# silverlight6/Ultrasound_Modeling

Hardware: AMD Instinct MI355X
Metric: segmentation training images/sec at 256x256 (higher is better)
Workload: dtype bf16

## Files before the change

ultrasound_modeling_amd/csrc/conv_big.hip:

```cpp
#include "common.h"

struct BigJob {
  const bf16_t* x;
  const bf16_t* w;
  void* y;
  const float* bias;
  const float* scale;
  const bf16_t* res;
  int32_t H, W, d, Hl, Wl, PH, PW, NV;
  int32_t tiles_x, tiles_per_v, npatches;
  int32_t ldx, ldy, ldr, Cin, nchunks, Nw, Kw, Nout, act;
  float alpha;
  int32_t out_f32, accumulate, flip;
  int32_t gx, gy, npa, nstages;
  uint32_t x_bytes, w_bytes;
  int32_t mask_ch;
  int32_t one_tap;
  uint16_t tapmask[4];
};
struct BigParams {
  BigJob job[4];
};

typedef __attribute__((address_space(3))) void* lds_ptr_t;
#define OOB_OFF 0x80000000u

template <int NT, int NS, int NW = 4>
__global__ __launch_bounds__(64 * NW) void conv_big_kernel(const BigParams P) {
#if defined(__HIP_DEVICE_COMPILE__)
  constexpr int BN = 16 * NT;
  constexpr int W_BYTES = 9 * BN * 64;
  constexpr int NPW = 9 * BN / 16;
  constexpr int W_IT = (NPW + NW - 1) / NW;
  constexpr int A_IT = ((NS * NW == 16 ? 36 : 18) + NW - 1) / NW;
  extern __shared__ __attribute__((aligned(1024))) char lds[];
  const BigJob& p = P.job[blockIdx.z];
  if ((int)blockIdx.x >= p.gx || (int)blockIdx.y >= p.gy) return;

  const int tid = threadIdx.x, lane = tid & 63, wv = __builtin_amdgcn_readfirstlane(tid >> 6);
  const int n0 = blockIdx.y * BN;
  const int HW2 = p.PW + 2, HPP = (p.PH + 2) * HW2, NHP = p.NV * HPP;
  const int a_bytes = p.npa * 1024, stage_bytes = a_bytes + W_BYTES;
  const int dd = p.d * p.d;
  const float r_hpp = fdiv_rcp(HPP), r_hw2 = fdiv_rcp(HW2), r_tpv = fdiv_rcp(p.tiles_per_v), r_tx = fdiv_rcp(p.tiles_x), r_dd = fdiv_rcp(dd),
              r_d = fdiv_rcp(p.d);

  const __amdgpu_buffer_rsrc_t rx = __builtin_amdgcn_make_buffer_rsrc((void*)p.x, 0, p.x_bytes, 0x00020000);
  const __amdgpu_buffer_rsrc_t rw = __builtin_amdgcn_make_buffer_rsrc((void*)p.w, 0, p.w_bytes, 0x00020000);
  const int slot_q = (lane & 3) ^ (((lane >> 4) & 1) << 1);
  uint32_t a_off[A_IT], w_off[W_IT];
#pragma unroll
  for (int it = 0; it < A_IT; ++it) {
    const int hp = 16 * (wv + NW * it) + (lane >> 2);
    uint32_t off = OOB_OFF;
    if (hp < NHP) {
      int pi, rem, hy, hx;
      fdivmod(hp, HPP, r_hpp, pi, rem);
      fdivmod(rem, HW2, r_hw2, hy, hx);
      int gp = blockIdx.x * p.NV + pi;
      if (gp < p.npatches) {
        int v, tt, ty, tx, b, ab, la, lb;
        fdivmod(gp, p.tiles_per_v, r_tpv, v, tt);
        fdivmod(tt, p.tiles_x, r_tx, ty, tx);
        fdivmod(v, dd, r_dd, b, ab);
        fdivmod(ab, p.d, r_d, la, lb);
        int ly = __mul24(ty, p.PH) + hy - 1, lx = __mul24(tx, p.PW) + hx - 1;
        if ((unsigned)ly < (unsigned)p.Hl && (unsigned)lx < (unsigned)p.Wl)
          off = (uint32_t)(__mul24(__mul24(__mul24(b, p.H) + la + __mul24(p.d, ly), p.W) + lb + __mul24(p.d, lx), p.ldx) + slot_q * 8) * 2u;
      }
    }
    a_off[it] = off;
  }
#pragma unroll
  for (int it = 0; it < W_IT; ++it) {
    const int row = 16 * (wv + NW * it) + (lane >> 2);
    uint32_t off = OOB_OFF;
    if (row < 9 * BN) {
      int t = row / BN, n = row - t * BN;
      int tw = p.flip ? 8 - t : t;
      if (p.one_tap) tw = t == 4 ? 0 : -1;
      if (tw >= 0 && n0 + n < p.Nw) off = (uint32_t)((n0 + n) * p.Kw + tw * p.Cin + slot_q * 8) * 2u;
    }
    w_off[it] = off;
  }
  const int cq = slot_q * 8;

  auto issue = [&](int ck, int stage) {
    char* abuf = lds + stage * stage_bytes;
    char* wbuf = abuf + a_bytes;
    const uint32_t cb = ck * 64;
    const bool cok = ck * 32 + cq < p.Cin;
#pragma unroll
    for (int it = 0; it < A_IT; ++it) {
      const int j = wv + NW * it;
      if (j < p.npa) {
        __builtin_amdgcn_raw_ptr_buffer_load_lds(rx, (lds_ptr_t)(abuf + j * 1024), 16, cok ? a_off[it] + cb : OOB_OFF, 0, 0, 0);
      }
    }
#pragma unroll
    for (int it = 0; it < W_IT; ++it) {
      const int j = wv + NW * it;
      if (j < NPW) {
        __builtin_amdgcn_raw_ptr_buffer_load_lds(rw, (lds_ptr_t)(wbuf + j * 1024), 16, cok ? w_off[it] + cb : OOB_OFF, 0, 0, 0);
      }
    }
  };

  issue(0, 0);
  const int pl = lane & 15, qk = lane >> 4;
  const int rows_per_strip = 16 / p.PW, spp = (p.PH * p.PW) >> 4;
  int hb[NS];
  int64_t opix[NS];
  bool ovalid[NS];
#pragma unroll
  for (int a = 0; a < NS; ++a) {
    int s = wv * NS + a;
    int pi, sl, r, c;
    fdivmod(s, spp, fdiv_rcp(spp), pi, sl);
    fdivmod(pl, p.PW, fdiv_rcp(p.PW), r, c);
    int row = sl * rows_per_strip + r;
    hb[a] = pi * HPP + row * HW2 + c;
    int gp = blockIdx.x * p.NV + pi;
    ovalid[a] = gp < p.npatches;
    int gpc = ovalid[a] ? gp : 0;
    int v, tt, ty, tx, b, ab, la, lb;
    fdivmod(gpc, p.tiles_per_v, r_tpv, v, tt);
    fdivmod(tt, p.tiles_x, r_tx, ty, tx);
    fdivmod(v, dd, r_dd, b, ab);
    fdivmod(ab, p.d, r_d, la, lb);
    int iy = la + __mul24(p.d, __mul24(ty, p.PH) + row), ix = lb + __mul24(p.d, __mul24(tx, p.PW) + c);
    opix[a] = (int64_t)(__mul24(__mul24(b, p.H) + iy, p.W) + ix);
  }
  const int w_lane = pl * 64 + ((qk ^ (((pl >> 2) & 1) << 1)) << 4);

  f32x4_t acc[NS][NT];
#pragma unroll
  for (int a = 0; a < NS; ++a)
#pragma unroll
    for (int b = 0; b < NT; ++b) acc[a][b] = (f32x4_t){0.f, 0.f, 0.f, 0.f};

  const bool dbuf = p.nstages == 2;
  for (int ck = 0; ck < p.nchunks; ++ck) {
    asm volatile("s_waitcnt vmcnt(0)" ::: "memory");
    __syncthreads();
    if (dbuf && ck + 1 < p.nchunks) issue(ck + 1, (ck + 1) & 1);
    const char* abuf = lds + (dbuf ? (ck & 1) * stage_bytes : 0);
    const char* wbuf = abuf + a_bytes + w_lane;
    const uint32_t tmask = p.one_tap ? 0x010u : (p.mask_ch ? p.tapmask[(p.flip ? ck * 32 : n0) / p.mask_ch] : 0x1ffu);
#pragma unroll
    for (int t = 0; t < 9; ++t) {
      if (!((tmask >> t) & 1u)) continue;
      const int toff = (t / 3) * HW2 + (t % 3);
      bf16x8_t xf[NS], wf[NT];
#pragma unroll
      for (int a = 0; a < NS; ++a) {
        const int hp = hb[a] + toff;
        xf[a] = *reinterpret_cast<const bf16x8_t*>(abuf + (hp << 6) + ((qk << 4) ^ ((hp & 4) << 3)));
      }
#pragma unroll
      for (int b = 0; b < NT; ++b) wf[b] = *reinterpret_cast<const bf16x8_t*>(wbuf + (t * BN + b * 16) * 64);
#pragma unroll
      for (int a = 0; a < NS; ++a)
#pragma unroll
        for (int b = 0; b < NT; ++b) acc[a][b] = __builtin_amdgcn_mfma_f32_16x16x32_bf16(wf[b], xf[a], acc[a][b], 0, 0, 0);
    }
    if (!dbuf && ck + 1 < p.nchunks) {
      __syncthreads();
      issue(ck + 1, 0);
    }
  }

  const EpiArgs e = {p.scale, p.bias, p.res, p.y, p.ldy, p.ldr, p.Nout, p.act, p.alpha, p.out_f32, p.accumulate};
  const int nbase = n0 + qk * 4;
  EpiConst<NT> ec;
  epi_const_load<NT>(ec, p.bias, nbase, p.Nout);
  conv_epilogue<NS, NT>(e, ec, acc, opix, ovalid, nbase);
#endif
}

template <int NT, int NS, bool RES = false>
__global__ __launch_bounds__(256, 2) void conv_stream_kernel(const BigParams P, const int fast_wait) {
#if defined(__HIP_DEVICE_COMPILE__)
  const BigJob& p = P.job[blockIdx.z];
  constexpr int BN = 16 * NT;
  constexpr int W_BYTES = 9 * BN * 64;
  constexpr int NPW = 9 * BN / 16;
  constexpr int A_IT = NS == 4 ? 6 : 3;
  constexpr int MAXG = 64;
  extern __shared__ __attribute__((aligned(1024))) char lds[];
  __shared__ int s_grp[MAXG][4];

  const int tid = threadIdx.x, lane = tid & 63, wv = __builtin_amdgcn_readfirstlane(tid >> 6);
  const int n0 = blockIdx.y * BN;
  const int HW2 = p.PW + 2, NHP = (p.PH + 2) * HW2;
  const int a_bytes = p.npa * 1024;
  char* const wlds = lds;
  char* const alds = lds + p.nchunks * W_BYTES;
  const int dd = p.d * p.d;
  const float r_nch = fdiv_rcp(p.nchunks);
  const float r_hw2 = fdiv_rcp(HW2), r_tpv = fdiv_rcp(p.tiles_per_v), r_tx = fdiv_rcp(p.tiles_x), r_dd = fdiv_rcp(dd), r_d = fdiv_rcp(p.d);

  const int ngroups = p.npatches;
  const int xcd = blockIdx.x & 7, wj = blockIdx.x >> 3, nj = gridDim.x >> 3;
  const int gpx = (ngroups + 7) >> 3;
  const int g_lo = xcd * gpx + wj;
  int g_hi = (xcd + 1) * gpx;
  if (g_hi > ngroups) g_hi = ngroups;
  int ng = g_lo < g_hi ? (g_hi - g_lo + nj - 1) / nj : 0;
  if (ng > MAXG) ng = MAXG;
  if (ng == 0) return;

  const __amdgpu_buffer_rsrc_t rx = __builtin_amdgcn_make_buffer_rsrc((void*)p.x, 0, p.x_bytes, 0x00020000);
  const __amdgpu_buffer_rsrc_t rw = __builtin_amdgcn_make_buffer_rsrc((void*)p.w, 0, p.w_bytes, 0x00020000);
  const int slot_q = (lane & 3) ^ (((lane >> 4) & 1) << 1);
  const int cq = slot_q * 8;

  for (int j = wv; j < p.nchunks * NPW; j += 4) {
    const int ck = j / NPW, r = j - ck * NPW;
    const int row = 16 * r + (lane >> 2);
    const int t = row / BN, n = row - t * BN;
    int tw = p.flip ? 8 - t : t;
    if (p.one_tap) tw = t == 4 ? 0 : -1;
    const bool ok = tw >= 0 && (n0 + n) < p.Nw && (ck * 32 + cq) < p.Cin;
    __builtin_amdgcn_raw_ptr_buffer_load_lds(rw, (lds_ptr_t)(wlds + j * 1024), 16,
                                             ok ? (uint32_t)((n0 + n) * p.Kw + tw * p.Cin + ck * 32 + cq) * 2u : OOB_OFF, 0, 0, 0);
  }
  for (int i = tid; i < ng; i += 256) {
    const int g = g_lo + i * nj;
    int v, tt, ty, tx, b, ab, la, lb;
    fdivmod(g, p.tiles_per_v, r_tpv, v, tt);
    fdivmod(tt, p.tiles_x, r_tx, ty, tx);
    fdivmod(v, dd, r_dd, b, ab);
    fdivmod(ab, p.d, r_d, la, lb);
    const int64_t org = (((int64_t)(b * p.H + la + p.d * (ty * p.PH - 1))) * p.W + lb + p.d * (tx * p.PW - 1)) * p.ldx * 2;
    s_grp[i][0] = (int)(uint32_t)org;
    s_grp[i][1] = (b * p.H + la + p.d * ty * p.PH) * p.W + lb + p.d * tx * p.PW;
    s_grp[i][2] = ty * p.PH - 1;
    s_grp[i][3] = tx * p.PW - 1;
  }
  uint32_t a_rel[A_IT];
  int a_hy[A_IT], a_hx[A_IT];
#pragma unroll
  for (int it = 0; it < A_IT; ++it) {
    const int hp = 16 * (wv + 4 * it) + (lane >> 2);
    int hy, hx;
    fdivmod(hp, HW2, r_hw2, hy, hx);
    a_hy[it] = hp < NHP ? hy : -(1 << 20);
    a_hx[it] = hx;
    a_rel[it] = (uint32_t)(((p.d * hy) * p.W + p.d * hx) * p.ldx + cq) * 2u;
  }
  const int pl = lane & 15, qk = lane >> 4;
  const int rows_per_strip = 16 / p.PW;
  int hb[NS], orel[NS];
#pragma unroll
  for (int a = 0; a < NS; ++a) {
    const int sl = wv * NS + a;
    int r, c;
    fdivmod(pl, p.PW, fdiv_rcp(p.PW), r, c);
    const int row = sl * rows_per_strip + r;
    hb[a] = row * HW2 + c;
    orel[a] = p.d * row * p.W + p.d * c;
  }
  const int w_lane = pl * 64 + ((qk ^ (((pl >> 2) & 1) << 1)) << 4);
  const EpiArgs e = {p.scale, p.bias, p.res, p.y, p.ldy, p.ldr, p.Nout, p.act, p.alpha, p.out_f32, p.accumulate};
  const int nbase = n0 + qk * 4;
  EpiConst<NT> ec;
  epi_const_load<NT>(ec, p.bias, nbase, p.Nout);
  __syncthreads();

  auto issue_a = [&](int s) {
    const int gl = __builtin_amdgcn_readfirstlane(fdiv(s, r_nch)), ck = s - gl * p.nchunks;
    char* abuf = alds + (s & 1) * a_bytes;
    const uint32_t org = (uint32_t)s_grp[gl][0] + ck * 64;
    const int lym1 = s_grp[gl][2], lxm1 = s_grp[gl][3];
    const bool cok = ck * 32 + cq < p.Cin;
#pragma unroll
    for (int it = 0; it < A_IT; ++it) {
      const int j = wv + 4 * it;
      if (j < p.npa) {
        const bool ok = cok && (unsigned)(lym1 + a_hy[it]) < (unsigned)p.Hl && (unsigned)(lxm1 + a_hx[it]) < (unsigned)p.Wl;
        __builtin_amdgcn_raw_ptr_buffer_load_lds(rx, (lds_ptr_t)(abuf + j * 1024), 16, ok ? org + a_rel[it] : OOB_OFF, 0, 0, 0);
      }
    }
  };

  f32x4_t acc[NS][NT];
  const int total = ng * p.nchunks;
  issue_a(0);
  for (int s = 0; s < total; ++s) {
    const int gl = __builtin_amdgcn_readfirstlane(fdiv(s, r_nch)), ck = s - gl * p.nchunks;
    if (fast_wait && s > 0 && ck == 0) asm volatile("s_waitcnt vmcnt(%0) lgkmcnt(0)\n\ts_barrier" ::"n"(NS * NT) : "memory");
    else asm volatile("s_waitcnt vmcnt(0) lgkmcnt(0)\n\ts_barrier" ::: "memory");
    uint2 rr[RES ? NS : 1][RES ? NT : 1];
    if constexpr (RES) {
      if (ck == p.nchunks - 1) {
        const int ob = s_grp[gl][1];
#pragma unroll
        for (int a = 0; a < NS; ++a)
#pragma unroll
          for (int b = 0; b < NT; ++b) {
            const int n = nbase + b * 16;
            rr[a][b] = *reinterpret_cast<const uint2*>(p.res + (int64_t)(ob + orel[a]) * p.ldr + (n < p.Nout ? n : 0));
          }
      }
    }
    if (s + 1 < total) issue_a(s + 1);
    if (ck == 0) {
#pragma unroll
      for (int a = 0; a < NS; ++a)
#pragma unroll
        for (int b = 0; b < NT; ++b) acc[a][b] = (f32x4_t){0.f, 0.f, 0.f, 0.f};
    }
    const char* abuf = alds + (s & 1) * a_bytes;
    const char* wbuf = wlds + ck * W_BYTES + w_lane;
    auto do_tap = [&](int t) {
      const int toff = (t / 3) * HW2 + (t % 3);
      bf16x8_t xf[NS], wf[NT];
#pragma unroll
      for (int a = 0; a < NS; ++a) {
        const int hp = hb[a] + toff;
        xf[a] = *reinterpret_cast<const bf16x8_t*>(abuf + (hp << 6) + ((qk << 4) ^ ((hp & 4) << 3)));
      }
#pragma unroll
      for (int b = 0; b < NT; ++b) wf[b] = *reinterpret_cast<const bf16x8_t*>(wbuf + (t * BN + b * 16) * 64);
#pragma unroll
      for (int a = 0; a < NS; ++a)
#pragma unroll
        for (int b = 0; b < NT; ++b) acc[a][b] = __builtin_amdgcn_mfma_f32_16x16x32_bf16(wf[b], xf[a], acc[a][b], 0, 0, 0);
    };
    if constexpr (RES || NT == 4) {
#pragma unroll
      for (int t = 0; t < 9; ++t) do_tap(t);
    } else if (p.one_tap) do_tap(4);
    else {
#pragma unroll
      for (int t = 0; t < 9; ++t) do_tap(t);
    }
    if (ck != p.nchunks - 1) continue;
    int64_t opix[NS];
    bool ovalid[NS];
    const int obase = s_grp[gl][1];
#pragma unroll
    for (int a = 0; a < NS; ++a) { opix[a] = obase + orel[a]; ovalid[a] = true; }
    if constexpr (RES) {
      const float alpha = p.alpha;
      const int act = p.act;
#pragma unroll
      for (int a = 0; a < NS; ++a) {
        bf16_t* const yrow = reinterpret_cast<bf16_t*>(p.y) + opix[a] * p.ldy;
#pragma unroll
        for (int b = 0; b < NT; ++b) {
          const int n = nbase + b * 16;
          if (n >= p.Nout) continue;
          const float v0 = apply_act(acc[a][b][0] + ec.bb[b].x, act, alpha) + __uint_as_float(rr[a][b].x << 16);
          const float v1 = apply_act(acc[a][b][1] + ec.bb[b].y, act, alpha) + __uint_as_float(rr[a][b].x & 0xffff0000u);
          const float v2 = apply_act(acc[a][b][2] + ec.bb[b].z, act, alpha) + __uint_as_float(rr[a][b].y << 16);
          const float v3 = apply_act(acc[a][b][3] + ec.bb[b].w, act, alpha) + __uint_as_float(rr[a][b].y & 0xffff0000u);
          uint2 o;
          o.x = pack2bf(v0, v1);
          o.y = pack2bf(v2, v3);
          *reinterpret_cast<uint2*>(yrow + n) = o;
        }
      }
    } else {
      conv_epilogue<NS, NT, true>(e, ec, acc, opix, ovalid, nbase);
    }
  }
#endif
}

static int big_fill_job(BigJob& p, const ConvPass& g, int PX, int any_cin = 0) {
  const int min_cin = knob<K_BIG_MIN_CIN>();
  const int B = g.B, H = g.H, W = g.W, d = g.d, ldx = g.ldx;
  if (d < 1 || H % d || W % d || (g.Cin < min_cin && !any_cin)) return 0;
  const int Hl = H / d, Wl = W / d;
  int PW;
  if (Wl % 16 == 0) PW = 16;
  else if (Wl == 8 || Wl == 4) PW = Wl;
  else return 0;
  int PH = PX / PW;
  if (PH > Hl) PH = Hl;
  if (Hl % PH || (PH * PW) % 16 || PX % (PH * PW)) return 0;
  const int NV = PX / (PH * PW);
  const int NHP = NV * (PH + 2) * (PW + 2);
  if (NHP > (PX == 256 ? 576 : 288)) return 0;
  if ((int64_t)B * H * W * ldx >= (1ll << 30) || (int64_t)g.Nw * g.Kw >= (1ll << 30)) return 0;
  if ((int64_t)B * H * W >= (1ll << 23) || (int64_t)B * d * d * (Hl / PH) * (Wl / PW) >= (1ll << 20)) return 0;
  p = {};
  p.x = g.x; p.w = g.w; p.y = g.y; p.bias = g.bias; p.scale = g.scale; p.res = g.res;
  p.H = H; p.W = W; p.d = d; p.Hl = Hl; p.Wl = Wl; p.PH = PH; p.PW = PW; p.NV = NV;
  p.tiles_x = Wl / PW;
  p.tiles_per_v = (Hl / PH) * p.tiles_x;
  p.npatches = B * d * d * p.tiles_per_v;
  p.ldx = ldx; p.ldy = g.ldy; p.ldr = g.ldr; p.Cin = g.Cin; p.nchunks = (g.Cin + 31) / 32;
  p.Nw = g.Nw; p.Kw = g.Kw; p.Nout = g.Nout; p.act = g.act; p.alpha = g.alpha; p.out_f32 = g.out_f32; p.accumulate = g.accumulate; p.flip = g.flip;
  p.gx = (p.npatches + NV - 1) / NV;
  p.x_bytes = (uint32_t)((int64_t)B * H * W * ldx * 2);
  p.w_bytes = (uint32_t)((int64_t)g.Nw * g.Kw * 2);
  p.npa = (NHP + 15) / 16;
  p.mask_ch = g.mask.group_ch;
  for (int c = 0; c < 4; ++c) p.tapmask[c] = g.mask.mask[c];
  p.one_tap = g.one_tap;
  return 1;
}

static int nt_for(int nout) { return nout <= 16 ? 1 : (nout <= 32 ? 2 : 4); }

template <int NT, int NS, int NW = 4>
static void big_launch_t(const BigParams& P, dim3 grid, size_t dyn, hipStream_t s) {
  if (usseg_lds_opt_in((const void*)conv_big_kernel<NT, NS, NW>, 160 * 1024)) return;
  hipLaunchKernelGGL((conv_big_kernel<NT, NS, NW>), grid, dim3(64 * NW), dyn, s, P);
}

static void big_launch(BigParams& P, int njobs, int nt, int PX, hipStream_t s, int w8 = 0) {
  int gx = 0, gy = 0, npa = 0;
  for (int j = 0; j < njobs; ++j) {
    BigJob& p = P.job[j];
    p.gy = (p.Nout + 16 * nt - 1) / (16 * nt);
    if (p.gx > gx) gx = p.gx;
    if (p.gy > gy) gy = p.gy;
    if (p.npa > npa) npa = p.npa;
  }
  const int stages_env = knob<K_BIG_STAGES>();
  int64_t total_wg = 0;
  for (int j = 0; j < njobs; ++j) total_wg += (int64_t)P.job[j].gx * P.job[j].gy;
  const int nstages = stages_env == 2 ? 2 : (stages_env == 1 ? 1 : (total_wg <= 512 ? 2 : 1));
  for (int j = 0; j < njobs; ++j) { P.job[j].npa = npa; P.job[j].nstages = nstages; }
  const size_t dyn = nstages * ((size_t)npa * 1024 + (size_t)9 * 16 * nt * 64);
  const dim3 grid(gx, gy, njobs);
  const int slot = usseg_prof_start(1, s);
  if (PX == 256 && w8) {
    if (nt == 1) big_launch_t<1, 2, 8>(P, grid, dyn, s);
    else if (nt == 2) big_launch_t<2, 2, 8>(P, grid, dyn, s);
    else big_launch_t<4, 2, 8>(P, grid, dyn, s);
  } else if (PX == 256) {
    if (nt == 1) big_launch_t<1, 4>(P, grid, dyn, s);
    else if (nt == 2) big_launch_t<2, 4>(P, grid, dyn, s);
    else big_launch_t<4, 4>(P, grid, dyn, s);
  } else {
    if (nt == 1) big_launch_t<1, 2>(P, grid, dyn, s);
    else if (nt == 2) big_launch_t<2, 2>(P, grid, dyn, s);
    else big_launch_t<4, 2>(P, grid, dyn, s);
  }
  usseg_prof_stop(1, slot, s);
}

template <int NT, int NS, bool RES = false>
static void stream_launch_t(const BigParams& P, dim3 grid, size_t dyn, int fast_wait, hipStream_t s) {
  if (usseg_lds_opt_in((const void*)conv_stream_kernel<NT, NS, RES>, 158 * 1024)) return;
  hipLaunchKernelGGL((conv_stream_kernel<NT, NS, RES>), grid, dim3(256), dyn, s, P, fast_wait);
}

struct StreamPlan {
  BigJob job;
  int nt, PX, res, fast_wait;
  size_t dyn;
  unsigned wgx, gy;
};
static int stream_plan(const ConvPass& g, StreamPlan& sp) {
  const int mode = knob<K_STREAM>();
  const int px_env = knob<K_STREAM_PX>();
  const int min_steps = knob<K_STREAM_MIN_STEPS>();
  const int wgx_env = knob<K_STREAM_WGX>();
  const int occ_env = knob<K_STREAM_OCC>();
  if (!mode || g.mask.group_ch) return 0;
  const int res_env = knob<K_STREAM_RES>();
  if (g.out_f32 || g.accumulate || g.scale) return 0;
  if (g.res && (!res_env || (g.ldr & 3))) return 0;
  const int nt = nt_for(g.Nout);
  const int nchunks = (g.Cin + 31) / 32;
  const size_t wbytes = (size_t)nchunks * 9 * 16 * nt * 64;
  if (wbytes > 40960) return 0;
  const int gy = (g.Nout + 16 * nt - 1) / (16 * nt);
  BigJob& p = sp.job;
  for (int PX = 256; PX >= 128; PX >>= 1) {
    if (px_env && PX != px_env) continue;
    if (!big_fill_job(p, g, PX, 1)) continue;
    if (p.NV != 1 || p.PW != 16) continue;
    if (g.one_tap && (nt == 4 || g.res)) return 0;
    const size_t dyn = wbytes + 2 * (size_t)p.npa * 1024;
    int occ = (int)((160 * 1024 - 2048) / (dyn + 1024));
    if (occ > 4) occ = 4;
    if (occ_env > 0 && occ_env < occ) occ = occ_env;
    if (occ < 1) continue;
    int wgx = (256 * occ / gy) & ~7;
    if (wgx < 8) wgx = 8;
    if (wgx_env >= 8) wgx = wgx_env & ~7;
    const int gpx = (p.npatches + 7) / 8;
    int per_wg = (gpx + wgx / 8 - 1) / (wgx / 8);
    if (per_wg * nchunks < min_steps && !px_env) continue;
    if (per_wg > 64) { wgx = ((gpx + 63) / 64) * 8; per_wg = 64; }
    sp.fast_wait = g.Nout % (16 * nt) == 0 && !g.res;
    sp.nt = nt; sp.PX = PX; sp.res = g.res != nullptr; sp.dyn = dyn; sp.wgx = (unsigned)wgx; sp.gy = (unsigned)gy;
    return 1;
  }
  return 0;
}
static void stream_launch(const StreamPlan* sp, int n, hipStream_t s) {
  BigParams P;
  for (int j = 0; j < n; ++j) P.job[j] = sp[j].job;
  for (int j = n; j < 4; ++j) P.job[j] = sp[0].job;
  const dim3 grid(sp[0].wgx, sp[0].gy, (unsigned)n);
  const int nt = sp[0].nt, PX = sp[0].PX, fast_wait = sp[0].fast_wait;
  const size_t dyn = sp[0].dyn;
  const int slot = usseg_prof_start(1, s);
  if (sp[0].res) {
    if (PX == 256) {
      if (nt == 1) stream_launch_t<1, 4, true>(P, grid, dyn, fast_wait, s);
      else if (nt == 2) stream_launch_t<2, 4, true>(P, grid, dyn, fast_wait, s);
      else stream_launch_t<4, 4, true>(P, grid, dyn, fast_wait, s);
    } else {
      if (nt == 1) stream_launch_t<1, 2, true>(P, grid, dyn, fast_wait, s);
      else if (nt == 2) stream_launch_t<2, 2, true>(P, grid, dyn, fast_wait, s);
      else stream_launch_t<4, 2, true>(P, grid, dyn, fast_wait, s);
    }
  } else if (PX == 256) {
    if (nt == 1) stream_launch_t<1, 4>(P, grid, dyn, fast_wait, s);
    else if (nt == 2) stream_launch_t<2, 4>(P, grid, dyn, fast_wait, s);
    else stream_launch_t<4, 4>(P, grid, dyn, fast_wait, s);
  } else {
    if (nt == 1) stream_launch_t<1, 2>(P, grid, dyn, fast_wait, s);
    else if (nt == 2) stream_launch_t<2, 2>(P, grid, dyn, fast_wait, s);
    else stream_launch_t<4, 2>(P, grid, dyn, fast_wait, s);
  }
  usseg_prof_stop(1, slot, s);
}
static bool stream_same_plan(const StreamPlan& a, const StreamPlan& b) {
  return a.nt == b.nt && a.PX == b.PX && a.res == b.res && a.fast_wait == b.fast_wait && a.dyn == b.dyn && a.wgx == b.wgx && a.gy == b.gy;
}

int usseg_try_launch_conv_big(const ConvPass* g, int njobs, hipStream_t s) {
  const int mode = knob<K_BIG>();
  const int px_env = knob<K_BIG_PX>();
  const int nt_env = knob<K_BIG_NT>();
  const int min_wg = knob<K_BIG_MIN_WG>();
  const int wg_min = knob<K_BIG_WG_TILE>();
  if (!mode || njobs < 1 || njobs > 4) return 0;
  {
    const int multi = knob<K_STREAM_MULTI>();
    const int merge = knob<K_STREAM_MERGE>();
    bool all = (njobs == 1 || multi) && njobs <= 4;
    StreamPlan sp[4];
    for (int j = 0; j < njobs && all; ++j) all = stream_plan(g[j], sp[j]) != 0;
    if (all) {
      for (int j = 0; j < njobs;) {
        int n = 1;
        while (merge && j + n < njobs && stream_same_plan(sp[j], sp[j + n])) ++n;
        stream_launch(sp + j, n, s);
        j += n;
      }
      return 1;
    }
  }
  int nt_max = 1;
  for (int j = 0; j < njobs; ++j) nt_max = nt_for(g[j].Nout) > nt_max ? nt_for(g[j].Nout) : nt_max;
  BigParams P;
  int best_px = 0, best_nt = 0;
  int64_t best_wg = 0;
  for (int PX = 256; PX >= 128 && !best_px; PX >>= 1) {
    if (px_env && PX != px_env) continue;
    bool ok = true;
    for (int j = 0; j < njobs && ok; ++j) ok = big_fill_job(P.job[j], g[j], PX);
    if (!ok) continue;
    for (int nt = nt_max; nt >= 1; nt >>= 1) {
      if (nt_env && nt != nt_env) continue;
      int64_t wg = 0;
      for (int j = 0; j < njobs; ++j) wg += (int64_t)P.job[j].gx * ((P.job[j].Nout + 16 * nt - 1) / (16 * nt));
      if (PX == 256 && !px_env) {
        if (nt == nt_max && wg >= 2048) { best_px = PX; best_nt = nt; best_wg = wg; }
        break;
      }
      best_px = PX; best_nt = nt; best_wg = wg;
      if (wg >= wg_min || nt_env) break;
    }
  }
  if (!best_px || (best_wg < min_wg && !(px_env || nt_env))) return 0;
  int w8 = 0;
  {
    const int w8_mode = knob<K_BIG_W8>();
    const int w8_min = knob<K_BIG_W8_MIN>();
    if (w8_mode && best_px == 128) {
      bool ok = true;
      int64_t wg = 0;
      for (int j = 0; j < njobs && ok; ++j) {
        ok = big_fill_job(P.job[j], g[j], 256);
        if (ok) wg += (int64_t)P.job[j].gx * ((P.job[j].Nout + 16 * best_nt - 1) / (16 * best_nt));
      }
      if (ok && ((wg >= w8_min && best_nt == 4) || w8_mode == 2)) { w8 = 1; best_px = 256; }
    }
  }
  for (int j = 0; j < njobs; ++j)
    if (!big_fill_job(P.job[j], g[j], best_px)) return 0;
  if (g[0].mask.group_ch && (njobs != 1 || g[0].mask.group_ch % (g[0].flip ? 32 : 16 * best_nt))) return 0;
  big_launch(P, njobs, best_nt, best_px, s, w8);
  return 1;
}
```

ultrasound_modeling_amd/csrc/knobs.h:

```cpp
#pragma once
#include <stdint.h>
#include <stdlib.h>

#define USSEG_KNOBS(X)                                                                                                                  \
                                                                                                                      \
  X(K_BIG,                "USSEG_BIG",                INT,     1,     ONCE,     "0: conv_big and the streaming conv take no launch")        \
  X(K_BIG_PX,             "USSEG_BIG_PX",             INT,     0,     ONCE,     "conv_big: force the pixel tile (128 / 256; 0: planner)")   \
  X(K_BIG_NT,             "USSEG_BIG_NT",             INT,     0,     ONCE,     "conv_big: force the channel tile (1 / 2 / 4 x 16; 0: planner)") \
  X(K_BIG_MIN_WG,         "USSEG_BIG_MIN_WG",         INT,     128,   ONCE,     "conv_big: smallest launch it takes, in workgroups")        \
  X(K_BIG_WG_TILE,        "USSEG_BIG_WG_TILE",        INT,     512,   ONCE,     "conv_big: narrow the channel tile below this many workgroups") \
  X(K_BIG_MIN_CIN,        "USSEG_BIG_MIN_CIN",        INT,     33,    ONCE,     "conv_big: fewest input channels of a pass it takes")       \
  X(K_BIG_STAGES,         "USSEG_BIG_STAGES",         INT,     0,     ONCE,     "conv_big LDS stages: 0 by launch size, 1 / 2 forced")      \
  X(K_BIG_W8,             "USSEG_BIG_W8",             INT,     1,     PER_CALL, "256-pixel tile on eight waves: 0 never, 1 planner, 2 forced") \
  X(K_BIG_W8_MIN,         "USSEG_BIG_W8_MIN",         INT,     128,   ONCE,     "fewest workgroups left for the eight-wave tile")           \
  X(K_STREAM,             "USSEG_STREAM",             INT,     1,     ONCE,     "0: the streaming conv takes no launch")                    \
  X(K_STREAM_PX,          "USSEG_STREAM_PX",          INT,     0,     ONCE,     "streaming conv: force the pixel tile (128 / 256; 0: planner)") \
  X(K_STREAM_MIN_STEPS,   "USSEG_STREAM_MIN_STEPS",   INT,     1,     PER_CALL, "streaming conv: fewest K steps per workgroup it takes")    \
  X(K_STREAM_WGX,         "USSEG_STREAM_WGX",         INT,     0,     PER_CALL, "streaming conv: force grid.x (>= 8, rounded down to a multiple of 8)") \
  X(K_STREAM_OCC,         "USSEG_STREAM_OCC",         INT,     0,     ONCE,     "streaming conv: cap on workgroups per CU (0: by LDS)")     \
  X(K_STREAM_RES,         "USSEG_STREAM_RES",         INT,     1,     ONCE,     "0: passes with a residual do not stream")                  \
  X(K_STREAM_MULTI,       "USSEG_STREAM_MULTI",       INT,     1,     ONCE,     "0: multi-job launches do not stream")                      \
  X(K_STREAM_MERGE,       "USSEG_STREAM_MERGE",       INT,     1,     PER_CALL, "streaming jobs of one plan in one launch (0: a launch per job)") \
                                                                                                     \
  X(K_NO_HALO,            "USSEG_NO_HALO",            PRESENT, 0,     ONCE,     "the halo-tile conv and weight-gradient kernels take no launch") \
  X(K_NO_PERSIST,         "USSEG_NO_PERSIST",         PRESENT, 0,     ONCE,     "conv_halo: never the persistent variant")                  \
  X(K_PERSIST_OCC,        "USSEG_PERSIST_OCC",        INT,     0,     ONCE,     "persistent conv_halo: workgroups per CU (0: by LDS)")      \
                                                                                                                    \
  X(K_IGEMM_WG_MIN,       "USSEG_IGEMM_WG_MIN",       INT,     256,   ONCE,     "igemm: narrow the channel tile below this many workgroups") \
  X(K_IGEMM_KC,           "USSEG_IGEMM_KC",           INT,     0,     ONCE,     "register-staged igemm: force the K step (4 / 8 chunks; 0: by K length)") \
  X(K_IGEMM_DMA,          "USSEG_IGEMM_DMA",          INT,     1,     ONCE,     "0: never the LDS-DMA igemm")                               \
  X(K_IGEMM_DMA_MIN,      "USSEG_IGEMM_DMA_MIN",      INT,     4,     ONCE,     "LDS-DMA igemm: fewest K chunks it takes")                  \
  X(K_IGEMM_DMA_BATCHED,  "USSEG_IGEMM_DMA_BATCHED",  INT,     1,     ONCE,     "0: batched GEMMs stay on the register-staged igemm")       \
  X(K_IGEMM_XCD,          "USSEG_IGEMM_XCD",          INT,     1,     ONCE,     "XCD-aware item order: 0 off, 1 activation-heavy launches, 2 all") \
  X(K_IGEMM_PERSIST,      "USSEG_IGEMM_PERSIST",      INT,     1,     ONCE,     "0: never the persistent LDS-DMA igemm")                    \
  X(K_IGEMM_STAGES8,      "USSEG_IGEMM_STAGES8",      INT,     4,     ONCE,     "ring depth of sparse long-K 128-channel launches (2: off, 3, 4)") \
  X(K_IGEMM_STAGES8_WG,   "USSEG_IGEMM_STAGES8_WG",   INT,     256,   ONCE,     "largest launch, in workgroups, that gets the deeper ring") \
                                                                                                         \
  X(K_WGRAD_DMA,          "USSEG_WGRAD_DMA",          INT,     1,     ONCE,     "0: never the LDS-DMA per-tap weight gradient / batched TN GEMM") \
  X(K_WGRAD_TM,           "USSEG_WGRAD_TM",           INT,     0,     ONCE,     "per-tap wgrad: force the tile (1: 64x64, 2: 128x128; 0: planner)") \
  X(K_WGD_TARGET,         "USSEG_WGD_TARGET",         INT,     512,   ONCE,     "per-tap wgrad: workgroups the split-K aims for")           \
  X(K_WGD_CAP,            "USSEG_WGD_CAP",            INT,     4,     ONCE,     "per-tap wgrad: slab traffic cap, in multiples of the operand bytes") \
  X(K_WG_QUANT,           "USSEG_WG_QUANT",           INT,     1,     ONCE,     "0: no wave-quantisation search of the split count (both wgrad kernels)") \
  X(K_WGRAD_DEBUG,        "USSEG_WGRAD_DEBUG",        PRESENT, 0,     ONCE,     "print every weight-gradient plan to stderr")               \
  X(K_WGRAD_POW2,         "USSEG_WGRAD_POW2",         INT,     1,     ONCE,     "0: no shift decode of power-of-two grids")                 \
  X(K_WGRAD_XCD,          "USSEG_WGRAD_XCD",          INT,     1,     ONCE,     "0: no XCD-aware item order in the per-tap wgrad")          \
  X(K_WG_TARGET,          "USSEG_WG_TARGET",          INT,     256,   ONCE,     "halo wgrad: workgroups the split-K aims for")              \
  X(K_SLAB_CAP,           "USSEG_SLAB_CAP",           INT,     2,     ONCE,     "halo wgrad: slab traffic cap, in multiples of the operand bytes") \
  X(K_WGHALO_XCD,         "USSEG_WGHALO_XCD",         INT,     1,     ONCE,     "0: no XCD-aware item order in the halo wgrad")             \
  X(K_WGRAD_PF,           "USSEG_WGRAD_PF",           INT,     1,     ONCE,     "0: halo wgrad without the register prefetch")              \
  X(K_WGRAD_8W,           "USSEG_WGRAD_8W",           INT,     1,     ONCE,     "0: the 64x64 halo wgrad tile on four waves, not eight")    \
  X(K_TCONV_HALO,         "USSEG_TCONV_HALO",         INT,     0,     PER_CALL, "1: transposed-conv wgrad as four parity-class halo jobs")  \
                                                                                                                      \
  X(K_CARD_BWD_G,         "USSEG_CARD_BWD_G",         INT,     0,     ONCE,     "fused cardinal backward: force the workgroup pairs (0: one resident wave)") \
  X(K_LN_TILE,            "USSEG_LN_TILE",            INT,     1,     ONCE,     "0: never the tile LayerNorm backward")                     \
  X(K_LN_PAIR,            "USSEG_LN_PAIR",            INT,     1,     ONCE,     "0: never the paired LayerNorm backward launch")            \
  X(K_LN_TILE_MIN,        "USSEG_LN_TILE_MIN",        INT,     32768, ONCE,     "fewest pixels for the tile / paired LayerNorm backward")   \
                                                                                     \
  X(K_FLASH_TILE,         "USSEG_FLASH_TILE",         INT,     -1,    ONCE,     "fused attention tiling 0 / 1 / 2 (-1: by problem size)")   \
  X(K_WINATTN_MFMA,       "USSEG_WINATTN_MFMA",       INT,     1,     ONCE,     "0: window attention without the MFMA kernels")             \
  X(K_LOSS_PPT,           "USSEG_LOSS_PPT",           INT,     4,     ONCE,     "softmax + loss kernel: pixels per thread")

enum Knob {
#define X(id, name, kind, def, life, doc) id,
  USSEG_KNOBS(X)
#undef X
};
enum { KNOB_INT, KNOB_PRESENT, KNOB_ONCE, KNOB_PER_CALL };
struct KnobDef { const char* name; int kind; int64_t def; int life; };
constexpr KnobDef kKnobs[] = {
#define X(id, name, kind, def, life, doc) {name, KNOB_##kind, def, KNOB_##life},
  USSEG_KNOBS(X)
#undef X
};

template <Knob K>
__attribute__((visibility("hidden"))) inline int64_t knob() {
  auto read = [] {
    const char* v = getenv(kKnobs[K].name);
    return kKnobs[K].kind == KNOB_PRESENT ? (int64_t)(v != nullptr) : (v ? (int64_t)atoll(v) : kKnobs[K].def);
  };
  if constexpr (kKnobs[K].life == KNOB_PER_CALL) return read();
  else {
    static const int64_t v = read();
    return v;
  }
}
```

Baseline: 5527.

## Prefetch LDS fragments ahead of MFMAs in narrow streaming conv tiles

Adds a software-pipelined path for the streaming conv kernel (non-residual, NT<=2). It preloads all nine tap weight fragments and a sliding window of input fragments, reusing input rows across kernel rows, and interleaves the LDS reads with MFMAs using sched_barriers. The aim is to hide LDS latency and cut redundant fragment reads. It uses more registers and could hurt occupancy. A default-on knob selects it.

```diff
diff --git a/ultrasound_modeling_amd/csrc/conv_big.hip b/ultrasound_modeling_amd/csrc/conv_big.hip
--- a/ultrasound_modeling_amd/csrc/conv_big.hip
+++ b/ultrasound_modeling_amd/csrc/conv_big.hip
@@ -1,3 +1,5 @@
+#include <type_traits>
+
 #include "common.h"
 
 struct BigJob {
@@ -179,7 +181,7 @@
 }
 
 template <int NT, int NS, bool RES = false>
-__global__ __launch_bounds__(256, 2) void conv_stream_kernel(const BigParams P, const int fast_wait) {
+__global__ __launch_bounds__(256, 2) void conv_stream_kernel(const BigParams P, const int fast_wait, const int frag_ahead) {
 #if defined(__HIP_DEVICE_COMPILE__)
   const BigJob& p = P.job[blockIdx.z];
   constexpr int BN = 16 * NT;
@@ -284,88 +286,143 @@
     }
   };
 
-  f32x4_t acc[NS][NT];
-  const int total = ng * p.nchunks;
-  issue_a(0);
-  for (int s = 0; s < total; ++s) {
-    const int gl = __builtin_amdgcn_readfirstlane(fdiv(s, r_nch)), ck = s - gl * p.nchunks;
-    if (fast_wait && s > 0 && ck == 0) asm volatile("s_waitcnt vmcnt(%0) lgkmcnt(0)\n\ts_barrier" ::"n"(NS * NT) : "memory");
-    else asm volatile("s_waitcnt vmcnt(0) lgkmcnt(0)\n\ts_barrier" ::: "memory");
-    uint2 rr[RES ? NS : 1][RES ? NT : 1];
-    if constexpr (RES) {
-      if (ck == p.nchunks - 1) {
-        const int ob = s_grp[gl][1];
+  constexpr bool AHEAD_OK = !RES && NT <= 2;
+  auto run = [&](auto ahead_c) {
+    constexpr bool AH = decltype(ahead_c)::value;
+    int xa[AH ? 4 : 1];
+    if constexpr (AH) {
+#pragma unroll
+      for (int m = 0; m < 4; ++m) {
+        const int hp = hb[0] + m;
+        xa[m] = (hp << 6) + ((qk << 4) ^ ((hp & 4) << 3));
+      }
+    }
+    f32x4_t acc[NS][NT];
+    const int total = ng * p.nchunks;
+    issue_a(0);
+    for (int s = 0; s < total; ++s) {
+      const int gl = __builtin_amdgcn_readfirstlane(fdiv(s, r_nch)), ck = s - gl * p.nchunks;
+      if (fast_wait && s > 0 && ck == 0) asm volatile("s_waitcnt vmcnt(%0) lgkmcnt(0)\n\ts_barrier" ::"n"(NS * NT) : "memory");
+      else asm volatile("s_waitcnt vmcnt(0) lgkmcnt(0)\n\ts_barrier" ::: "memory");
+      uint2 rr[RES ? NS : 1][RES ? NT : 1];
+      if constexpr (RES) {
+        if (ck == p.nchunks - 1) {
+          const int ob = s_grp[gl][1];
+#pragma unroll
+          for (int a = 0; a < NS; ++a)
+#pragma unroll
+            for (int b = 0; b < NT; ++b) {
+              const int n = nbase + b * 16;
+              rr[a][b] = *reinterpret_cast<const uint2*>(p.res + (int64_t)(ob + orel[a]) * p.ldr + (n < p.Nout ? n : 0));
+            }
+        }
+      }
+      if (s + 1 < total) issue_a(s + 1);
+      if (ck == 0) {
 #pragma unroll
         for (int a = 0; a < NS; ++a)
+#pragma unroll
+          for (int b = 0; b < NT; ++b) acc[a][b] = (f32x4_t){0.f, 0.f, 0.f, 0.f};
+      }
+      const int a_off = (s & 1) * a_bytes;
+      const char* abuf = alds + a_off;
+      const char* wbuf = wlds + ck * W_BYTES + w_lane;
+      auto do_tap = [&](int t) {
+        const int toff = (t / 3) * HW2 + (t % 3);
+        bf16x8_t xf[NS], wf[NT];
+#pragma unroll
+        for (int a = 0; a < NS; ++a) {
+          const int hp = hb[a] + toff;
+          xf[a] = *reinterpret_cast<const bf16x8_t*>(abuf + (hp << 6) + ((qk << 4) ^ ((hp & 4) << 3)));
+        }
+#pragma unroll
+        for (int b = 0; b < NT; ++b) wf[b] = *reinterpret_cast<const bf16x8_t*>(wbuf + (t * BN + b * 16) * 64);
+#pragma unroll
+        for (int a = 0; a < NS; ++a)
+#pragma unroll
+          for (int b = 0; b < NT; ++b) acc[a][b] = __builtin_amdgcn_mfma_f32_16x16x32_bf16(wf[b], xf[a], acc[a][b], 0, 0, 0);
+      };
+      if constexpr (RES || NT == 4) {
+#pragma unroll
+        for (int t = 0; t < 9; ++t) do_tap(t);
+      } else if (p.one_tap) do_tap(4);
+      else if constexpr (AH) {
+        bf16x8_t xf[NS + 2][3], wf[9][NT];
+        auto load_x = [&](int j, int kc) {
+          const int m = (2 * j + kc) & 7, off = a_off + xa[m & 3];
+          xf[j][kc] = *reinterpret_cast<const bf16x8_t*>(alds + (m < 4 ? off : off ^ 32) + 64 * (18 * j + kc - (m & 3)));
+        };
+        auto load_w = [&](int t) {
+#pragma unroll
+          for (int b = 0; b < NT; ++b) wf[t][b] = *reinterpret_cast<const bf16x8_t*>(wbuf + (t * BN + b * 16) * 64);
+        };
+#pragma unroll
+        for (int kc = 0; kc < 3; ++kc) {
+          load_w(kc);
+#pragma unroll
+          for (int j = 0; j < NS; ++j) load_x(j, kc);
+          __builtin_amdgcn_sched_barrier(0);
+        }
+#pragma unroll
+        for (int kr = 0; kr < 3; ++kr)
+#pragma unroll
+          for (int kc = 0; kc < 3; ++kc) {
+#pragma unroll
+            for (int a = 0; a < NS; ++a) {
+#pragma unroll
+              for (int b = 0; b < NT; ++b)
+                acc[a][b] = __builtin_amdgcn_mfma_f32_16x16x32_bf16(wf[kr * 3 + kc][b], xf[a + kr][kc], acc[a][b], 0, 0, 0);
+              if (a == 0 && kr < 2) {
+                __builtin_amdgcn_sched_barrier(0);
+                load_x(NS + kr, kc);
+                __builtin_amdgcn_sched_barrier(0);
+              }
+            }
+            if (kr < 2) {
+              __builtin_amdgcn_sched_barrier(0);
+              load_w(kr * 3 + kc + 3);
+              __builtin_amdgcn_sched_barrier(0);
+            }
+          }
+      } else {
+#pragma unroll
+        for (int t = 0; t < 9; ++t) do_tap(t);
+      }
+      if (ck != p.nchunks - 1) continue;
+      int64_t opix[NS];
+      bool ovalid[NS];
+      const int obase = s_grp[gl][1];
+#pragma unroll
+      for (int a = 0; a < NS; ++a) { opix[a] = obase + orel[a]; ovalid[a] = true; }
+      if constexpr (RES) {
+        const float alpha = p.alpha;
+        const int act = p.act;
+#pragma unroll
+        for (int a = 0; a < NS; ++a) {
+          bf16_t* const yrow = reinterpret_cast<bf16_t*>(p.y) + opix[a] * p.ldy;
 #pragma unroll
           for (int b = 0; b < NT; ++b) {
             const int n = nbase + b * 16;
-            rr[a][b] = *reinterpret_cast<const uint2*>(p.res + (int64_t)(ob + orel[a]) * p.ldr + (n < p.Nout ? n : 0));
+            if (n >= p.Nout) continue;
+            const float v0 = apply_act(acc[a][b][0] + ec.bb[b].x, act, alpha) + __uint_as_float(rr[a][b].x << 16);
+            const float v1 = apply_act(acc[a][b][1] + ec.bb[b].y, act, alpha) + __uint_as_float(rr[a][b].x & 0xffff0000u);
+            const float v2 = apply_act(acc[a][b][2] + ec.bb[b].z, act, alpha) + __uint_as_float(rr[a][b].y << 16);
+            const float v3 = apply_act(acc[a][b][3] + ec.bb[b].w, act, alpha) + __uint_as_float(rr[a][b].y & 0xffff0000u);
+            uint2 o;
+            o.x = pack2bf(v0, v1);
+            o.y = pack2bf(v2, v3);
+            *reinterpret_cast<uint2*>(yrow + n) = o;
           }
-      }
-    }
-    if (s + 1 < total) issue_a(s + 1);
-    if (ck == 0) {
-#pragma unroll
-      for (int a = 0; a < NS; ++a)
-#pragma unroll
-        for (int b = 0; b < NT; ++b) acc[a][b] = (f32x4_t){0.f, 0.f, 0.f, 0.f};
-    }
-    const char* abuf = alds + (s & 1) * a_bytes;
-    const char* wbuf = wlds + ck * W_BYTES + w_lane;
-    auto do_tap = [&](int t) {
-      const int toff = (t / 3) * HW2 + (t % 3);
-      bf16x8_t xf[NS], wf[NT];
-#pragma unroll
-      for (int a = 0; a < NS; ++a) {
-        const int hp = hb[a] + toff;
-        xf[a] = *reinterpret_cast<const bf16x8_t*>(abuf + (hp << 6) + ((qk << 4) ^ ((hp & 4) << 3)));
-      }
-#pragma unroll
-      for (int b = 0; b < NT; ++b) wf[b] = *reinterpret_cast<const bf16x8_t*>(wbuf + (t * BN + b * 16) * 64);
-#pragma unroll
-      for (int a = 0; a < NS; ++a)
-#pragma unroll
-        for (int b = 0; b < NT; ++b) acc[a][b] = __builtin_amdgcn_mfma_f32_16x16x32_bf16(wf[b], xf[a], acc[a][b], 0, 0, 0);
-    };
-    if constexpr (RES || NT == 4) {
-#pragma unroll
-      for (int t = 0; t < 9; ++t) do_tap(t);
-    } else if (p.one_tap) do_tap(4);
-    else {
-#pragma unroll
-      for (int t = 0; t < 9; ++t) do_tap(t);
-    }
-    if (ck != p.nchunks - 1) continue;
-    int64_t opix[NS];
-    bool ovalid[NS];
-    const int obase = s_grp[gl][1];
-#pragma unroll
-    for (int a = 0; a < NS; ++a) { opix[a] = obase + orel[a]; ovalid[a] = true; }
-    if constexpr (RES) {
-      const float alpha = p.alpha;
-      const int act = p.act;
-#pragma unroll
-      for (int a = 0; a < NS; ++a) {
-        bf16_t* const yrow = reinterpret_cast<bf16_t*>(p.y) + opix[a] * p.ldy;
-#pragma unroll
-        for (int b = 0; b < NT; ++b) {
-          const int n = nbase + b * 16;
-          if (n >= p.Nout) continue;
-          const float v0 = apply_act(acc[a][b][0] + ec.bb[b].x, act, alpha) + __uint_as_float(rr[a][b].x << 16);
-          const float v1 = apply_act(acc[a][b][1] + ec.bb[b].y, act, alpha) + __uint_as_float(rr[a][b].x & 0xffff0000u);
-          const float v2 = apply_act(acc[a][b][2] + ec.bb[b].z, act, alpha) + __uint_as_float(rr[a][b].y << 16);
-          const float v3 = apply_act(acc[a][b][3] + ec.bb[b].w, act, alpha) + __uint_as_float(rr[a][b].y & 0xffff0000u);
-          uint2 o;
-          o.x = pack2bf(v0, v1);
-          o.y = pack2bf(v2, v3);
-          *reinterpret_cast<uint2*>(yrow + n) = o;
         }
-      }
-    } else {
-      conv_epilogue<NS, NT, true>(e, ec, acc, opix, ovalid, nbase);
-    }
-  }
+      } else {
+        conv_epilogue<NS, NT, true>(e, ec, acc, opix, ovalid, nbase);
+      }
+    }
+  };
+  if constexpr (AHEAD_OK) {
+    if (frag_ahead) run(std::true_type{});
+    else run(std::false_type{});
+  } else run(std::false_type{});
 #endif
 }
 
@@ -447,8 +504,9 @@
 
 template <int NT, int NS, bool RES = false>
 static void stream_launch_t(const BigParams& P, dim3 grid, size_t dyn, int fast_wait, hipStream_t s) {
+  const int frag_ahead = !RES && NT <= 2 && knob<K_FRAG_AHEAD>() != 0;
   if (usseg_lds_opt_in((const void*)conv_stream_kernel<NT, NS, RES>, 158 * 1024)) return;
-  hipLaunchKernelGGL((conv_stream_kernel<NT, NS, RES>), grid, dim3(256), dyn, s, P, fast_wait);
+  hipLaunchKernelGGL((conv_stream_kernel<NT, NS, RES>), grid, dim3(256), dyn, s, P, fast_wait, frag_ahead);
 }
 
 struct StreamPlan {
diff --git a/ultrasound_modeling_amd/csrc/knobs.h b/ultrasound_modeling_amd/csrc/knobs.h
--- a/ultrasound_modeling_amd/csrc/knobs.h
+++ b/ultrasound_modeling_amd/csrc/knobs.h
@@ -21,6 +21,7 @@
   X(K_STREAM_RES,         "USSEG_STREAM_RES",         INT,     1,     ONCE,     "0: passes with a residual do not stream")                  \
   X(K_STREAM_MULTI,       "USSEG_STREAM_MULTI",       INT,     1,     ONCE,     "0: multi-job launches do not stream")                      \
   X(K_STREAM_MERGE,       "USSEG_STREAM_MERGE",       INT,     1,     PER_CALL, "streaming jobs of one plan in one launch (0: a launch per job)") \
+  X(K_FRAG_AHEAD,         "USSEG_FRAG_AHEAD",         INT,     1,     ONCE,     "0: the narrow streaming conv tiles read each LDS fragment right before its MFMA") \
                                                                                                      \
   X(K_NO_HALO,            "USSEG_NO_HALO",            PRESENT, 0,     ONCE,     "the halo-tile conv and weight-gradient kernels take no launch") \
   X(K_NO_PERSIST,         "USSEG_NO_PERSIST",         PRESENT, 0,     ONCE,     "conv_halo: never the persistent variant")                  \
```

Measured after the change: 5580, median of 6. Within noise of the previous version (+1.0%).
